# s22s/erased-cells

Measured on AMD Instinct MI355X. Metric: Gcells/s + HBM-GB/s roofline %, u8/u16->f64 16384^2, 1/2/4/8 GPUs, higher is better.
Workload: dtype f64

## Files before the change

### erased-cells_amd/csrc/ec_abi.hip

```cpp
#include <hip/hip_runtime.h>


#include <cfloat>
#include <cstdarg>
#include <cstdio>
#include <cstring>
#include <map>
#include <mutex>
#include <string>

#include "ec_lattice.hpp"
#include "ec_map_kernels.hpp"
#include "ec_reduce_kernels.hpp"
#include "ec_runtime.hpp"

namespace ecd {

static_assert(kMaxReduceBlocks <= kFinalizeMaxParts, "the finalize kernels read at most kFinalizeMaxParts partials");

static ec_status ensure_init() { return ensure_ready(); }

static int64_t* result_words(const Scratch& sc) { return sc.host_dev ? sc.host_dev : sc.dev_result(); }
static ec_status fetch_result(const Scratch& sc, int words, hipStream_t s) {
    if (!sc.host_dev) {
// ... 14 lines not shown
    return st;
}

template <typename K>
static int resident_per_cu(K kernel, int block, int want) {
    int nb = 0;
    if (hipOccupancyMaxActiveBlocksPerMultiprocessor(&nb, kernel, block, 0) != hipSuccess || nb < 1) {
        (void)hipGetLastError();
        return want;
    }
    return nb < want ? nb : want;
}

static unsigned residue(const void* p, size_t mod) { return static_cast<unsigned>(reinterpret_cast<uintptr_t>(p) % mod); }
static ReducePlan plan_reduction(const void* p0, unsigned residue1, size_t cell_size, size_t n, const ReduceShape& shape,
                                 const size_t* stream_bytes, int nstreams) {
    return reduce_plan(residue(p0, 16), residue1, cell_size, n, shape, device_cus(), tuning().reduce_bpc, tuning().unaligned_vector != 0,
                       cache_plan(stream_bytes, nstreams));
}
constexpr ReduceShape kScanShape = {kRBlock, kReduceU, 4, kRBlock, 4};

static inline hipStream_t S(ec_stream s) { return static_cast<hipStream_t>(s); }

template <typename Fn> struct pure_store : std::false_type {};
template <typename W> struct pure_store<FillFn<W>> : std::true_type {};

template <typename Fn, int U>
static void launch_map_u(const Fn& fn, size_t n, hipStream_t s) {
    const size_t groups = n / Fn::CPL;
    const size_t tiles = (groups + size_t(kBlock) * U - 1) / (size_t(kBlock) * U);
    const size_t stream_bytes[2] = {n * Fn::kIn0, n * Fn::kIn1};
    const unsigned lds = (pure_store<Fn>::value ? static_cast<unsigned>(tuning().write_lds_kb.load())
                                                : (Fn::kIn0 != 0 ? static_cast<unsigned>(tuning().map_lds_kb.load()) : 0u)) << 10;
    k_map<Fn, U><<<grid_for(tiles), kBlock, lds, s>>>(fn, n, cache_plan(stream_bytes, 2));
}

template <typename Fn>
static ec_status launch_map(const Fn& fn, size_t n, bool aligned, hipStream_t s, const char* what) {
    if (n == 0) return EC_OK;
    if (!aligned) {
        k_map_cellwise<Fn><<<grid_capped((n + kBlock - 1) / kBlock, 8), kBlock, 0, s>>>(fn, n);
    } else {
        switch (tuning().map_u) {
            case 1: launch_map_u<Fn, 1>(fn, n, s); break;
            case 4: launch_map_u<Fn, 4>(fn, n, s); break;
            default: launch_map_u<Fn, 2>(fn, n, s); break;
        }
    }
    return check_launch(what);
// ... 29 lines not shown
        break;
    switch (st) { EC_WITH_CT(EC_ROW) }
#undef EC_ROW
    return set_error(EC_ERR_UNSUPPORTED_TYPE, "convert: bad dtype");
}

template <typename T>
static ec_status launch_min_max(const void* p, const uint8_t* mask, size_t n, int64_t* keys2_dev, hipStream_t s) {
    Scratch sc;
    ec_status st = get_scratch(s, &sc);
    if (st != EC_OK) return st;
    const T* tp = static_cast<const T*>(p);
    unsigned grid = 0;
    if (n > 0) {
        const size_t stream_bytes[2] = {n * sizeof(T), mask ? n : 0};
        auto launch = [&](auto u_tag, auto block_tag, int per_cu) {
            constexpr int U = decltype(u_tag)::value, BLOCK = decltype(block_tag)::value;
            static const int resident[2] = {resident_per_cu(k_min_max_partials<T, false, U, BLOCK>, BLOCK, per_cu),
                                            resident_per_cu(k_min_max_partials<T, true, U, BLOCK>, BLOCK, per_cu)};
            const ReduceShape shape = {BLOCK, U, resident[mask ? 1 : 0], kBlock, 8};
            const ReducePlan pl = plan_reduction(p, mask ? residue(mask, 16 / sizeof(T)) : 0u, sizeof(T), n, shape, stream_bytes, 2);
            grid = pl.grid;
            int64_t* direct = pl.aligned && pl.single ? keys2_dev : nullptr;
            if (!pl.aligned) {
                if (mask) k_min_max_partials_cellwise<T, true><<<grid, kBlock, 0, s>>>(tp, mask, n, sc.dev);
                else k_min_max_partials_cellwise<T, false><<<grid, kBlock, 0, s>>>(tp, nullptr, n, sc.dev);
            } else if (mask) {
                k_min_max_partials<T, true, U, BLOCK><<<grid, BLOCK, 0, s>>>(tp, mask, n, sc.dev, pl.head_policy, direct);
            } else {
                k_min_max_partials<T, false, U, BLOCK><<<grid, BLOCK, 0, s>>>(tp, nullptr, n, sc.dev, pl.head_policy, direct);
            }
            return direct != nullptr;
        };
        using std::integral_constant;
        bool direct = false;
        switch (tuning().reduce_shape) {
// ... 237 lines not shown
extern "C" ec_status ec_min_max(ec_dtype t, const void* p, const uint8_t* mask_or_null, size_t n, ec_value* mn, ec_value* mx,
                                ec_stream stream) {
    EC_REQUIRE_INIT();
    if (!mn || !mx || (n > 0 && !p)) return set_error(EC_ERR_ARG, "ec_min_max: null pointer");
    int64_t keys2[2];
    ec_status st = sync_result(S(stream), 2, keys2, [&](const Scratch&, int64_t* words) {
        return dispatch_min_max(t, p, mask_or_null, n, words, S(stream));
    });
    if (st != EC_OK) return st;
    return ec_min_max_decode(t, keys2, mn, mx);
}

template <typename W>
static ec_status first_diff_w(const void* l, const void* r, size_t n, const Scratch& sc, hipStream_t s, unsigned* grid_out) {
    const size_t stream_bytes[2] = {n * sizeof(W), n * sizeof(W)};
    const ReducePlan pl = plan_reduction(l, residue(r, 16), sizeof(W), n, kScanShape, stream_bytes, 2);
    k_first_diff_partials<W, kReduceU><<<pl.grid, kRBlock, 0, s>>>(static_cast<const W*>(l), static_cast<const W*>(r), n,
                                                                  reinterpret_cast<uint64_t*>(sc.dev), pl.aligned, pl.head_policy);
    *grid_out = pl.grid;
    return check_launch("first_diff(partials)");
}

extern "C" ec_status ec_first_difference(ec_dtype t, const void* l, const void* r, size_t n, uint64_t* index, ec_stream stream) {
    EC_REQUIRE_INIT();
    if (!ecl::valid(t)) return set_error(EC_ERR_UNSUPPORTED_TYPE, "ec_first_difference: bad dtype %d", int(t));
    if (!index || (n > 0 && (!l || !r))) return set_error(EC_ERR_ARG, "ec_first_difference: null pointer");
    *index = n;
    if (n == 0) return EC_OK;
    int64_t word[2];
    ec_status st = sync_result(S(stream), 1, word, [&](const Scratch& sc, int64_t* words) {
        unsigned grid = 0;
// ... 116 lines not shown
    if (n == 0) return EC_OK;
    if (!m || !out) return set_error(EC_ERR_ARG, "ec_mask_not: null pointer");
    MaskNot fn{m, out};
    return launch_map(fn, n, aligned16(m, out, out), S(stream), "mask_not");
}

extern "C" ec_status ec_mask_counts_device(const uint8_t* m, size_t n, uint64_t* counts2_dev, ec_stream stream) {
    EC_REQUIRE_INIT();
    if (!counts2_dev || (n > 0 && !m)) return set_error(EC_ERR_ARG, "ec_mask_counts_device: null pointer");
    Scratch sc;
    ec_status st = get_scratch(S(stream), &sc);
    if (st != EC_OK) return st;
    unsigned grid = 0;
    if (n > 0) {
        const size_t stream_bytes[1] = {n};
        const ReducePlan pl = plan_reduction(m, 0u, 1, n, kScanShape, stream_bytes, 1);
        grid = pl.grid;
        uint64_t* direct = pl.single ? counts2_dev : nullptr;
        const int one = tuning().counts_one_launch.load();
        uint64_t* acc = (!direct && ((one == 1 && n < (size_t(1) << 29)) || (one >= 2 && n < (size_t(1) << 40)))) ? reinterpret_cast<uint64_t*>(sc.dev_acc()) : nullptr;
        k_mask_count_partials<kReduceU><<<grid, kRBlock, 0, S(stream)>>>(m, n, reinterpret_cast<uint64_t*>(sc.dev), pl.aligned, pl.head_policy,
                                                                        direct, acc, counts2_dev);
        st = check_launch("mask_counts(partials)");
        if (st != EC_OK || direct || acc) return st;
    }
    k_mask_count_finalize<<<1, kFinalizeBlock, 0, S(stream)>>>(reinterpret_cast<const uint64_t*>(sc.dev), static_cast<int>(grid), n, counts2_dev);
    return check_launch("mask_counts(finalize)");
}

extern "C" ec_status ec_mask_counts(const uint8_t* m, size_t n, uint64_t* n_true, uint64_t* n_false, ec_stream stream) {
    EC_REQUIRE_INIT();
// ... 41 lines not shown
```

### erased-cells_amd/csrc/ec_binop_tu.hpp

```cpp
#pragma once

#include <hip/hip_runtime.h>

#include <cmath>

#include "ec_binop_kernels.hpp"
#include "ec_runtime.hpp"

namespace ecd {

static inline unsigned lds_cap(int knob, int rule_kb) { return static_cast<unsigned>(knob >= 0 ? knob : rule_kb) << 10; }

template <typename L, typename R, int OP>
static ec_status launch_binop_pair(const void* l, const void* r, size_t n, double* out, hipStream_t s) {
    const Tuning& tu = tuning();
    const L* lp = static_cast<const L*>(l);
    const R* rp = static_cast<const R*>(r);
    constexpr int U = kBinopU;
    if (!aligned16(l, r, out)) {
        k_binop_cellwise<L, R, OP><<<grid_capped((n + kBlock - 1) / kBlock, 8), kBlock, 0, s>>>(lp, rp, out, n);
        return check_launch("binop(cellwise)");
    }
    constexpr bool kCanStage = Staged<L>::value || Staged<R>::value;
    const int variant = tu.binop_variant.load();
    const size_t stream_bytes[2] = {n * sizeof(L), l == r ? 0 : n * sizeof(R)};
    unsigned policy = cache_plan(stream_bytes, 2, n * sizeof(double));
    if (l == r && (policy & 1u)) policy |= 2u;
    constexpr bool kRulePair = kCanStage && ((sizeof(L) == 8) != (sizeof(R) == 8)) && (sizeof(L) <= 4 || sizeof(R) <= 4);
    const bool by_rule = variant < 0 && kRulePair && policy == 0 && n >= (size_t(1) << 20);
    if (kCanStage && (variant == 1 || by_rule)) {
        const size_t tiles = (n / kLdsWaveCells + kWavesPerBlock - 1) / kWavesPerBlock;
        constexpr unsigned kStatic = kWavesPerBlock * unsigned(Staged<L>::kSlabBytes + Staged<R>::kSlabBytes);
        const int knob = tu.binop_lds_kb.load();
        const unsigned lds = knob >= 0 ? unsigned(knob) << 10 : by_rule ? 32000u - kStatic : 0u;
        k_binop_lds<L, R, OP><<<grid_for(tiles), kBlock, lds, s>>>(lp, rp, out, n);
        if (by_rule) lds_rule_launches().fetch_add(1, std::memory_order_relaxed);
        return check_launch(by_rule ? "binop(lds, by rule)" : "binop(lds)");
    }
    const LoadedStream st[2] = {{l, sizeof(L)}, {r, sizeof(R)}};
    const unsigned head = peel_head(st, 2, n);
    const size_t tiles = (((n - head) >> 1) + size_t(kBlock) * U - 1) / (size_t(kBlock) * U);
    k_binop_direct<L, R, OP, U><<<grid_for(tiles), kBlock, lds_cap(tuning().binop_lds_kb.load(), sizeof(L) == 8 && sizeof(R) == 8 ? 48 : 0), s>>>(lp, rp, out, n, head | (policy << 8));
    return check_launch("binop(direct)");
}
// ... 7 lines not shown
    constexpr int U = kBinopU;
    if (!aligned16(l, r, out) || !aligned16(lm, rm, om)) {
        k_masked_binop_cellwise<L, R, OP><<<grid_capped((n + kBlock - 1) / kBlock, 8), kBlock, 0, s>>>(lp, lm, rp, rm, out, om, n);
        return check_launch("masked_binop(cellwise)");
    }
    constexpr bool kCanStage = Staged<L>::value || Staged<R>::value;
    if (kCanStage && tu.binop_variant == 1) {
        const size_t tiles = (n / kLdsWaveCells + kWavesPerBlock - 1) / kWavesPerBlock;
        k_masked_binop<L, R, OP, U, true><<<grid_for(tiles), kBlock, lds_cap(tu.binop_lds_kb.load(), 0), s>>>(lp, lm, rp, rm, out, om, n, 0u);
        return check_launch("masked_binop(lds)");
    }
    const LoadedStream st[2] = {{l, sizeof(L)}, {r, sizeof(R)}};
    const unsigned head = peel_head(st, 2, n);
    const size_t tiles = (((n - head) >> 1) + size_t(kBlock) * U - 1) / (size_t(kBlock) * U);
    const size_t stream_bytes[4] = {n * sizeof(L), l == r ? 0 : n * sizeof(R), n, lm == rm ? 0 : n};
    unsigned policy = cache_plan(stream_bytes, 4, n * sizeof(double));
    if (l == r && (policy & 1u)) policy |= 2u;
    if (lm == rm && (policy & 4u)) policy |= 8u;
    k_masked_binop<L, R, OP, U, false><<<grid_for(tiles), kBlock, 0, s>>>(lp, lm, rp, rm, out, om, n, head | (policy << 8));
    return check_launch("masked_binop(direct)");
}


template <typename L, int OP>
static ec_status launch_scalar(const void* l, double rhs, size_t n, double* out, hipStream_t s) {
    const L* lp = static_cast<const L*>(l);
    constexpr int U = kBinopU;
    if (!aligned16(l, out, out)) {
        k_binop_scalar_cellwise<L, OP><<<grid_capped((n + kBlock - 1) / kBlock, 8), kBlock, 0, s>>>(lp, rhs, out, n);
        return check_launch("binop_scalar(cellwise)");
    }
    const LoadedStream st[1] = {{l, sizeof(L)}};
    const unsigned head = peel_head(st, 1, n);
    const size_t tiles = (((n - head) >> 1) + size_t(kBlock) * U - 1) / (size_t(kBlock) * U);
    const size_t stream_bytes[1] = {n * sizeof(L)};
    const unsigned policy = cache_plan(stream_bytes, 1, n * sizeof(double));
    const unsigned lds = lds_cap(tuning().scalar_lds_kb.load(), sizeof(L) == 8 ? 32 : 0);
    if constexpr (!is_fp<L>::value) {
        if (std::isfinite(rhs) && !(OP == EC_DIV && rhs == 0.0)) {
            k_binop_scalar_direct<L, OP, U, false><<<grid_for(tiles), kBlock, lds, s>>>(lp, rhs, out, n, head | (policy << 8));
            return check_launch("binop_scalar(direct, no NaN possible)");
        }
    }
    k_binop_scalar_direct<L, OP, U><<<grid_for(tiles), kBlock, lds, s>>>(lp, rhs, out, n, head | (policy << 8));
    return check_launch("binop_scalar(direct)");
}

template <int OP>
ec_status dispatch_binop(int lt, const void* l, int rt, const void* r, size_t n, double* out, hipStream_t s) {
#define EC_ROW(LID, LT)                                                                         \
    case LID:                                                                                   \
// ... 60 lines not shown
```

### erased-cells_amd/csrc/ec_expr.hip

```cpp
#include <hip/hip_runtime.h>

#include <atomic>
#include <cstdlib>
#include <cstring>

#include <limits>
#include <mutex>
#include <string>

#include "ec_expr.hpp"
#include "ec_expr_fixed.hpp"
#include "ec_expr_jit.hpp"
#include "ec_lattice.hpp"
#include "ec_runtime.hpp"

using namespace ecd;

static std::atomic<int64_t> g_interpreted{0};

namespace ecd {
int64_t expr_stat(const char* key, bool* known) {
    if (!std::strcmp(key, "expr_interp_launches")) {
        *known = true;
        return g_interpreted.load(std::memory_order_relaxed);
// ... 42 lines not shown
        for (int j = k + 1; j < n_steps && !read_later; ++j) {
            const int me = kRefReg0 + st.dst;
            if (j > k + 1 && (steps[j].a == me || steps[j].b == me)) read_later = true;
            if (steps[j].dst == st.dst) break;
        }
        if (!read_later) w |= kStepNoFile;
        ea.prog[k >> 2] |= w << (16 * (k & 3));
    }
    ea.nstreams = static_cast<int8_t>(n_streams);
    ea.nsteps = static_cast<int8_t>(n_steps);
    return EC_OK;
}

static ec_status prepare_expr(ExprArgs& ea, bool* aligned_out, int* cls, const ec_dtype* dt, const void* const* p, int32_t n_streams,
                              const uint8_t* const* masks, const ec_value* scalars, int32_t n_scalars, const ec_expr_step* steps,
                              int32_t n_steps, size_t n, const char* what) {
    ec_status pst = program_of(ea, dt, n_streams, n_scalars, steps, n_steps, what);
    if (pst != EC_OK) return pst;
    if (!p || (n_scalars > 0 && !scalars)) return set_error(EC_ERR_ARG, "%s: null pointer", what);
    bool aligned = true;
    LoadedStream st[kExprMaxStreams];
    for (int k = 0; k < n_streams; ++k) {
        if (!p[k]) return set_error(EC_ERR_ARG, "%s: stream %d is null", what, k);
        ea.p[k] = p[k];
        aligned = aligned && aligned_to(p[k], 16);
        st[k] = {p[k], ecl::size_of(dt[k])};
        for (int j = 0; j < k && st[k].same_as < 0; ++j)
            if (p[j] == p[k]) st[k].same_as = j;
        cls[k] = fused_class_index(st[k].size);
    }
    for (int k = n_streams; k < kExprMaxStreams; ++k) ea.p[k] = p[0];
    for (int k = 0; k < n_scalars; ++k) {
        if (!ecl::valid(scalars[k].dtype)) return set_error(EC_ERR_ARG, "%s: bad dtype of scalar %d", what, k);
        ea.sc[k] = ec_value_to_f64(&scalars[k]);
    }
    if (masks)
        for (int k = 0; k < n_streams; ++k) {
            const ec_status mst = add_mask(masks[k], k, what, ea.m, &ea.nmask, &aligned);
            if (mst != EC_OK) return mst;
        }
    *aligned_out = aligned;
    ea.head = static_cast<uint8_t>(peel_head(st, n_streams, n));
    ea.cacheable = static_cast<uint8_t>(stream_policy(st, ea.nmask, n));
    return EC_OK;
}

static ec_status launch_expr(const ec_dtype* dt, const void* const* p, int32_t n_streams, const uint8_t* const* masks,
                             const ec_value* scalars, int32_t n_scalars, const ec_expr_step* steps, int32_t n_steps, size_t n,
                             double* out, uint8_t* out_mask, hipStream_t s, const char* what) {
    ExprArgs ea{};
    bool aligned = true;
    int cls[kExprMaxStreams] = {0, 0, 0, 0};
    if (!out) return set_error(EC_ERR_ARG, "%s: null pointer", what);
    if (masks && !out_mask) return set_error(EC_ERR_ARG, "%s: null out_mask", what);
    ec_status pst = prepare_expr(ea, &aligned, cls, dt, p, n_streams, masks, scalars, n_scalars, steps, n_steps, n, what);
    if (pst != EC_OK) return pst;
    aligned = aligned && aligned_to(out, 16) && (!masks || aligned_to(out_mask, 16));
    if (!aligned) {
        ea.head = 0;
        k_expr_cellwise<0><<<grid_capped((n + kBlock - 1) / kBlock, 8), kBlock, 0, s>>>(ea, out, out_mask, n);
        return check_launch("expr(cellwise)");
    }
    bool fixed = false;
    ec_status fst = expr_fixed_launch(ea, n, out, out_mask, s, &fixed);
    if (fst != EC_OK) return fst;
    if (fixed) return check_launch("expr(ahead-of-time)");
    bool compiled = false;
    ec_status jst = expr_jit_launch(ea, n, out, out_mask, nullptr, s, &compiled);
    if (jst != EC_OK) return jst;
    if (compiled) return check_launch("expr(compiled)");
// ... 32 lines not shown

static ec_status expr_min_max_keys(const ec_dtype* dt, const void* const* p, const uint8_t* const* masks_or_null, int32_t n_streams,
                                   const ec_value* scalars, int32_t n_scalars, const ec_expr_step* steps, int32_t n_steps, size_t n,
                                   int64_t* keys2_dev, hipStream_t s, const char* what) {
    ec_status st;
    {
        ExprArgs probe{};
        if ((st = program_of(probe, dt, n_streams, n_scalars, steps, n_steps, what)) != EC_OK) return st;
    }
    if (!keys2_dev) return set_error(EC_ERR_ARG, "%s: null keys", what);
    if ((st = check_hip(hipMemcpyAsync(keys2_dev, kF64Identities, sizeof kF64Identities, hipMemcpyHostToDevice, s), "hipMemcpyAsync(keys)")) != EC_OK) return st;
    if (n == 0) return EC_OK;
    ExprArgs ea{};
    bool aligned = true;
    int cls[kExprMaxStreams] = {0, 0, 0, 0};
    if ((st = prepare_expr(ea, &aligned, cls, dt, p, n_streams, masks_or_null, scalars, n_scalars, steps, n_steps, n, what)) != EC_OK) return st;
    if (aligned) {
        bool compiled = false;
        if ((st = expr_jit_launch(ea, n, nullptr, nullptr, keys2_dev, s, &compiled)) != EC_OK) return st;
        if (compiled) return EC_OK;
    }
    void *tmp = nullptr, *tmask = nullptr;
    if ((st = ec_alloc_async(&tmp, n * sizeof(double), s)) != EC_OK) return st;
    if (masks_or_null && (st = ec_alloc_async(&tmask, n, s)) != EC_OK) {
        (void)ec_free_async(tmp, s);
        return st;
    }
    st = launch_expr(dt, p, n_streams, masks_or_null, scalars, n_scalars, steps, n_steps, n, static_cast<double*>(tmp), static_cast<uint8_t*>(tmask), s, what);
    if (st == EC_OK) st = ec_min_max_keys(EC_F64, tmp, static_cast<const uint8_t*>(tmask), n, keys2_dev, s);
    const std::string keep = st != EC_OK ? last_error_text() : std::string();
    (void)ec_free_async(tmp, s);
// ... 64 lines not shown
```

### erased-cells_amd/csrc/ec_fused.hip

```cpp
#include <hip/hip_runtime.h>

#include "ec_fused_any.hpp"
#include "ec_lattice.hpp"

using namespace ecd;

static ec_status launch_fused_any(FusedArgs& fa, int nops, size_t n, double* out, uint8_t* out_mask, hipStream_t s) {
    LoadedStream st[4];
    int cls[4];
    bool small = fa.o2 == EC_DIV && (fa.o1 == EC_ADD || fa.o1 == EC_SUB) && (fa.o3 == EC_ADD || fa.o3 == EC_SUB || fa.o3 == kOpNone);
    for (int k = 0; k < 4; ++k) {
        if (k < nops && !fa.is_sc[k] && fa.alias[k] == k) st[k] = {fa.p[k], ecl::size_of(fa.dt[k])};
        cls[k] = fused_class_index(st[k].size);
        if (k < nops) small = small && !fa.is_sc[k] && ecl::is_integral(fa.dt[k]) && ecl::size_of(fa.dt[k]) <= 2;
    }
    fa.small = small ? 1 : 0;
    fa.head = static_cast<uint8_t>(peel_head(st, 4, n));
    fa.cacheable = static_cast<uint8_t>(stream_policy(st, fa.nmask, n));
    FusedAnyKernel kern = nullptr;
    switch (cls[0]) {
        case 0: kern = fused_any_kernel<0>(cls[1], cls[2], cls[3]); break;
        case 1: kern = fused_any_kernel<1>(cls[1], cls[2], cls[3]); break;
        case 2: kern = fused_any_kernel<2>(cls[1], cls[2], cls[3]); break;
        case 3: kern = fused_any_kernel<4>(cls[1], cls[2], cls[3]); break;
        default: kern = fused_any_kernel<8>(cls[1], cls[2], cls[3]); break;
    }
    if (!kern) return set_error(EC_ERR_ARG, "ec_fused: no kernel for load classes %d %d %d %d", cls[0], cls[1], cls[2], cls[3]);
    launch_stream_tile<kFusedU>(kern, fa.head, n, s, fa, out, out_mask, n);
    return check_launch("fused(any)");
}

static ec_status launch_fused(int o1, int o2, int o3, const ec_dtype dt[4], const void* const p[4],
                              const uint8_t* const masks[4], const ec_value* scalars, size_t n, double* out,
// ... 89 lines not shown
```

### erased-cells_amd/csrc/ec_runtime.hip

```cpp
#include <hip/hip_runtime.h>

#include <atomic>
#include <cstdarg>
#include <cstdint>
#include <cstdio>
#include <cstdlib>
#include <cstring>
#include <map>
#include <memory>
#include <mutex>
#include <string>

#include "ec_hostpipe.hpp"
#include "ec_runtime.hpp"

namespace ecd {

static thread_local std::string t_err;
static thread_local int t_narrow_src = -1, t_narrow_dst = -1;

ec_status set_error(ec_status code, const char* fmt, ...) {
    char buf[512];
    va_list ap;
    va_start(ap, fmt);
// ... 55 lines not shown
    int device = -1;
    int cus = 256;
    hipMemPool_t pool = nullptr;
    std::map<hipStream_t, ScratchEntry> scratch;
};

constexpr size_t kMaxScratchPerDevice = 64;

static std::mutex g_mu;
static std::map<int, DeviceState> g_devs;
static std::atomic<int> g_default_device{-1};
static std::atomic<uint64_t> g_generation{1};
static std::atomic<uint64_t> g_stamp{0};
static std::atomic<int64_t> g_lds_rule_launches{0};
std::atomic<int64_t>& lds_rule_launches() { return g_lds_rule_launches; }
static std::atomic<int64_t> g_pool_allocs{0};
static Tuning g_tuning;

static thread_local int t_device = -1;
static thread_local uint64_t t_generation = 0;
static thread_local int t_active = -1;
static thread_local int t_cus = 256;

int64_t expr_stat(const char* key, bool* known);
void expr_jit_release();
Tuning& tuning() { return g_tuning; }

namespace {
enum class Out { Clamp, Refuse, Bool };
struct Knob {
    const char* key;
    std::atomic<int>* i;
    std::atomic<int64_t>* l;
    int64_t lo, hi;
    Out out;
    bool pow2 = false;
};
constexpr int64_t kMaxMiB = int64_t(1) << 20;
const Knob kKnobs[] = {
    {"binop_variant", &g_tuning.binop_variant, nullptr, -1, 1, Out::Refuse},
    {"reduce_bpc", &g_tuning.reduce_bpc, nullptr, 0, kMaxReduceBlocks, Out::Clamp},
// ... 335 lines not shown
    }
    return EC_OK;
}

extern "C" ec_status ec_stream_destroy(ec_stream s) {
    ec_status st = ec_release_stream(s);
    if (st != EC_OK) return st;
    return check_hip(hipStreamDestroy(S(s)), "hipStreamDestroy");
}
extern "C" ec_status ec_stream_sync(ec_stream s) { return check_hip(hipStreamSynchronize(S(s)), "hipStreamSynchronize"); }

extern "C" ec_status ec_stat_get(const char* key, int64_t* value) {
    if (!key || !value) return set_error(EC_ERR_ARG, "ec_stat_get: null argument");
    if (!std::strcmp(key, "pool_allocs")) *value = g_pool_allocs.load(std::memory_order_relaxed);
    else if (!std::strcmp(key, "binop_lds_rule_launches")) *value = g_lds_rule_launches.load(std::memory_order_relaxed);
    else if (!std::strncmp(key, "tune.", 5)) {
        const Knob* kn = knob_of(key + 5);
        if (!kn) return set_error(EC_ERR_ARG, "ec_stat_get: unknown knob '%s'", key + 5);
        *value = kn->i ? int64_t(kn->i->load()) : kn->l->load();
    } else if (!std::strcmp(key, "devices")) {
        std::lock_guard<std::mutex> lk(g_mu);
        *value = static_cast<int64_t>(g_devs.size());
    } else if (!std::strcmp(key, "scratch_streams")) {
        std::lock_guard<std::mutex> lk(g_mu);
        int64_t n = 0;
        for (auto& kv : g_devs) n += static_cast<int64_t>(kv.second.scratch.size());
        *value = n;
    } else {
        bool known = false;
        *value = expr_stat(key, &known);
// ... 26 lines not shown
```

### erased-cells_amd/csrc/ec_runtime.hpp

```cpp
#pragma once

#include <hip/hip_runtime.h>
#include <stddef.h>
#include <stdint.h>

#include <atomic>
#include <memory>
#include <mutex>
#include <string>

#include "ec_reduce_plan.hpp"
#include "erased_cells.h"

namespace ecd {

constexpr int kBinopU = 2;

struct Tuning;
Tuning& tuning();
struct Tuning {
    std::atomic<int> binop_variant{-1};
    std::atomic<int> reduce_bpc{0};
    std::atomic<int> reduce_shape{0};
    std::atomic<int> map_u{2};
    std::atomic<int> peel{1};
// ... 11 lines not shown
    std::atomic<int> fused_lds_kb{0};
    std::atomic<int> counts_one_launch{1};
    std::atomic<int> cache_force{-1};
    std::atomic<int64_t> pool_keep_mb{32768};
};

int device_cus();
int current_device();

ec_status ensure_ready();
ec_status set_error(ec_status code, const char* fmt, ...);
ec_status set_error_text(ec_status code, const std::string& text);
const std::string& last_error_text();
ec_status set_narrowing(int src, int dst);
std::atomic<int64_t>& lds_rule_launches();
ec_status check_launch(const char* what);
ec_status check_hip(hipError_t e, const char* what);

class DeviceScope {
    int32_t before_ = -1;
    const bool had_;

public:
    DeviceScope() : had_(ec_get_device(&before_) == EC_OK) {}
    DeviceScope(const DeviceScope&) = delete;
    DeviceScope& operator=(const DeviceScope&) = delete;
    ~DeviceScope() {
        if (!had_ || current_device() == before_) return;
        const std::string keep = last_error_text();
        (void)ec_set_device(before_);
// ... 16 lines not shown
struct LoadedStream {
    const void* p = nullptr;
    size_t size = 0;
    int same_as = -1;
};
inline unsigned peel_head(const LoadedStream* st, int count, size_t n) {
    if (n < 2 || !tuning().peel) return 0;
    unsigned c0 = 0, c1 = 0;
    for (int k = 0; k < count; ++k) {
        c0 += peel_cost(st[k].p, st[k].size, 0);
        c1 += peel_cost(st[k].p, st[k].size, 1);
    }
    return c1 < c0 ? 1u : 0u;
}

inline unsigned cache_plan(const size_t* bytes, int n, size_t value_out_bytes = 0) {
    const int forced = tuning().cache_force.load();
    if (forced >= 0) return static_cast<unsigned>(forced) & ((1u << (n < 8 ? n : 8)) - 1u);
    const size_t budget = static_cast<size_t>(tuning().mall_mb.load()) << 20;
    unsigned plan = 0;
    size_t used = 0, largest_taken = 0;
    bool taken[8] = {false, false, false, false, false, false, false, false};
    for (int round = 0; round < n && n <= 8; ++round) {
        int best = -1;
        for (int k = 0; k < n; ++k)
            if (!taken[k] && bytes[k] > 0 && (best < 0 || bytes[k] < bytes[best])) best = k;
        if (best < 0 || used + bytes[best] > budget) break;
        taken[best] = true;
        used += bytes[best];
        if (bytes[best] > largest_taken) largest_taken = bytes[best];
        plan |= 1u << best;
    }
    if (value_out_bytes > 0 && plan != 0)
        for (int k = 0; k < n && n <= 8; ++k)
            if (!taken[k] && bytes[k] > 0 && bytes[k] <= largest_taken) return 0;
    return plan;
}

inline unsigned stream_policy(const LoadedStream (&st)[4], int nmask, size_t n) {
    size_t bytes[8] = {0, 0, 0, 0, 0, 0, 0, 0};
    for (int k = 0; k < 4; ++k) bytes[k] = st[k].same_as < 0 ? n * st[k].size : 0;
    for (int j = 0; j < nmask; ++j) bytes[4 + j] = n;
    unsigned policy = cache_plan(bytes, 8, n * sizeof(double));
    for (int k = 0; k < 4; ++k)
        if (st[k].same_as >= 0) policy = (policy & ~(1u << k)) | (((policy >> st[k].same_as) & 1u) << k);
    return policy;
}

inline ec_status add_mask(const uint8_t* m, int k, const char* what, const uint8_t** ms, int8_t* nmask, bool* aligned) {
    if (!m) return set_error(EC_ERR_ARG, "%s: null mask %d", what, k);
    for (int j = 0; j < *nmask; ++j)
        if (ms[j] == m) return EC_OK;
    ms[(*nmask)++] = m;
    *aligned = *aligned && aligned_to(m, 16);
    return EC_OK;
}

inline unsigned grid_for(size_t tiles) {
// ... 31 lines not shown
```

### erased-cells_amd/csrc/ec_window.hip

```cpp
#include <hip/hip_runtime.h>

#include "ec_lattice.hpp"
#include "ec_runtime.hpp"
#include "ec_window_checks.hpp"
#include "ec_window_kernels.hpp"

namespace ecd {

static bool make_axis(uint64_t win, uint64_t out, WindowAxis* a) {
    a->q = win / out;
    a->r = win % out;
    a->out = out;
    if (out > (UINT64_MAX >> 2)) return false;
    const unsigned __int128 worst = (unsigned __int128)(2 * out) * a->r + win;
    if (worst > UINT64_MAX) return false;
    const uint64_t num = a->q * out + a->r;
    a->d0 = num / (2 * out);
    a->rem0 = num % (2 * out);
    return true;
}

static bool rows_aligned(const void* raster, const WindowGeom& g, size_t cell, const void* contiguous) {
    return ((reinterpret_cast<uintptr_t>(raster) + g.origin * cell) | (g.pitch * cell) | (g.w * cell) | reinterpret_cast<uintptr_t>(contiguous)) % 16 == 0;
}

template <int W, bool MASKED>
static ec_status launch_window(int kind, const WindowArgs& args, const WindowAxis* ax, const WindowAxis* ay, bool vector, hipStream_t s) {
    WindowArgs a = args;
    const size_t bytes[2] = {a.g.n * W, MASKED ? a.g.n : 0};
    a.cacheable = cache_plan(bytes, 2);
    if (!vector) {
        const uint64_t chunks = ((a.g.w + kBlock - 1) / kBlock) * (a.g.n / a.g.w);
        const WindowAxis id_x{1, 0, a.g.w, 0, a.g.w}, id_y{1, 0, a.g.n / a.g.w, 0, a.g.n / a.g.w};
        if (kind == kWinPut) k_window_cellwise<W, MASKED, true><<<grid_capped(chunks, 8), kBlock, 0, s>>>(a, id_x, id_y);
        else k_window_cellwise<W, MASKED, false><<<grid_capped(chunks, 8), kBlock, 0, s>>>(a, ax ? *ax : id_x, ay ? *ay : id_y);
        return check_launch("window(cell-wise)");
    }
    const uint64_t slots = (a.g.n + (16 / W) - 1) / (16 / W), per_tile = uint64_t(kBlock) * kWindowU;
    const unsigned grid = grid_for((slots + per_tile - 1) / per_tile);
    if (uint64_t(grid) * per_tile < slots) return set_error(EC_ERR_ARG, "window: more than 2^31 tiles");
    if (ax) k_window_nearest<W, MASKED><<<grid, kBlock, 0, s>>>(a, *ax, *ay);
    else if (kind == kWinPut) k_window_put<W, MASKED><<<grid, kBlock, 0, s>>>(a);
    else k_window_copy<W, MASKED><<<grid, kBlock, 0, s>>>(a);
    return check_launch(ax ? "window(nearest)" : kind == kWinPut ? "window(put)" : "window(copy)");
}
// ... 53 lines not shown
```

### erased-cells_amd/csrc/ec_window_resample.hip

```cpp
#include <hip/hip_runtime.h>

#include "ec_window_checks.hpp"
#include "ec_window_resample_kernels.hpp"

namespace ecd {

typedef unsigned __int128 u128;

static uint64_t gcd_u64(uint64_t a, uint64_t b) {
    while (b) {
        const uint64_t t = a % b;
        a = b;
        b = t;
    }
    return a;
}

static const char* make_resample_axis(int32_t alg, uint64_t win, uint64_t out, ResampleAxis* a) {
    if (alg == EC_RESAMPLE_AVERAGE) {
        if ((u128)win * out > UINT64_MAX) return "win * out";
        const uint64_t g = gcd_u64(win, out);
        *a = ResampleAxis{win / g, 0, out / g, win / g, 0, win - 1, 0, 0, 0, 0};
    } else {
        if ((u128)2 * out * win + out > UINT64_MAX) return "2 * out * win + out";
// ... 4 lines not shown
    a->c0 = a->add / a->den;
    a->f0 = a->add % a->den;
    return nullptr;
}

static uint64_t resample_tiles(uint64_t n, size_t cell) {
    const uint64_t per_slot = 16 / cell, slots = n / per_slot + (n % per_slot != 0), per_tile = uint64_t(kBlock) * kWindowU;
    return slots / per_tile + (slots % per_tile != 0);
}

template <typename T, bool MASKED>
static ec_status launch_resample(const ResampleArgs& args, uint64_t win_cells, hipStream_t s) {
    constexpr size_t W = sizeof(T);
    ResampleArgs a = args;
    const size_t bytes[2] = {win_cells * W, MASKED ? win_cells : 0};
    a.w.cacheable = cache_plan(bytes, 2);
    k_window_resample<T, MASKED><<<grid_for(resample_tiles(a.w.g.n, W)), kBlock, 0, s>>>(a);
    return check_launch("window(resample)");
}

static ec_status dispatch_resample(ec_dtype t, const ResampleArgs& a, uint64_t win_cells, hipStream_t s) {
    const bool masked = a.w.in_mask != nullptr;
    switch (t) {
#define X(code, T) \
    case code: return masked ? launch_resample<T, true>(a, win_cells, s) : launch_resample<T, false>(a, win_cells, s);
        EC_WITH_CT(X)
#undef X
        default: return set_error(EC_ERR_UNSUPPORTED_TYPE, "ec_window_resample: bad dtype %d", int(t));
    }
}

// ... 39 lines not shown
```

Before: 611.7.

## Admit reads to MALL cache only when the same buffer was recently read

Adds a per-device host-side ledger that tracks recently read address ranges, with a byte counter standing in for cache pressure. A stream is marked cacheable in the last-level cache only if the same range was read recently enough to still fit in the budget. Streams seen for the first time are read with the non-caching policy. This aims to keep one-shot streaming reads from polluting the MALL while keeping reuse across calls. The cost is a mutex and ring scan on the host for every launch, and cache decisions now depend on call history, with the ledger bypassed during graph capture.

Result: no change. 614.8, median of 6 (+0.5%).

```diff
diff --git a/erased-cells_amd/csrc/ec_abi.hip b/erased-cells_amd/csrc/ec_abi.hip
--- a/erased-cells_amd/csrc/ec_abi.hip
+++ b/erased-cells_amd/csrc/ec_abi.hip
@@ -52,9 +52,9 @@
 
 static unsigned residue(const void* p, size_t mod) { return static_cast<unsigned>(reinterpret_cast<uintptr_t>(p) % mod); }
 static ReducePlan plan_reduction(const void* p0, unsigned residue1, size_t cell_size, size_t n, const ReduceShape& shape,
-                                 const size_t* stream_bytes, int nstreams) {
+                                 const size_t* stream_bytes, const void* const* stream_base, int nstreams, hipStream_t s) {
     return reduce_plan(residue(p0, 16), residue1, cell_size, n, shape, device_cus(), tuning().reduce_bpc, tuning().unaligned_vector != 0,
-                       cache_plan(stream_bytes, nstreams));
+                       cache_plan(stream_bytes, stream_base, nstreams, s));
 }
 constexpr ReduceShape kScanShape = {kRBlock, kReduceU, 4, kRBlock, 4};
 
@@ -62,6 +62,14 @@
 
 template <typename Fn> struct pure_store : std::false_type {};
 template <typename W> struct pure_store<FillFn<W>> : std::true_type {};
+
+template <typename Fn> static void map_inputs(const Fn&, const void* (&)[2]) { static_assert(Fn::kIn0 == 0 && Fn::kIn1 == 0, "name the Fn's inputs"); }
+template <typename Sx, typename Dx> static void map_inputs(const ConvertFn<Sx, Dx>& f, const void* (&p)[2]) { p[0] = f.src; }
+template <typename T> static void map_inputs(const NegFn<T>& f, const void* (&p)[2]) { p[0] = f.src; }
+template <typename W> static void map_inputs(const MaskFromNodataFn<W>& f, const void* (&p)[2]) { p[0] = f.src; }
+template <typename W> static void map_inputs(const MaskSelectFn<W>& f, const void* (&p)[2]) { p[0] = f.src, p[1] = f.mask; }
+template <int KIND> static void map_inputs(const MaskBin<KIND>& f, const void* (&p)[2]) { p[0] = f.l, p[1] = f.r; }
+static void map_inputs(const MaskNot& f, const void* (&p)[2]) { p[0] = f.m; }
 
 template <typename Fn, int U>
 static void launch_map_u(const Fn& fn, size_t n, hipStream_t s) {
@@ -70,7 +78,9 @@
     const size_t stream_bytes[2] = {n * Fn::kIn0, n * Fn::kIn1};
     const unsigned lds = (pure_store<Fn>::value ? static_cast<unsigned>(tuning().write_lds_kb.load())
                                                 : (Fn::kIn0 != 0 ? static_cast<unsigned>(tuning().map_lds_kb.load()) : 0u)) << 10;
-    k_map<Fn, U><<<grid_for(tiles), kBlock, lds, s>>>(fn, n, cache_plan(stream_bytes, 2));
+    const void* stream_base[2] = {nullptr, nullptr};
+    map_inputs(fn, stream_base);
+    k_map<Fn, U><<<grid_for(tiles), kBlock, lds, s>>>(fn, n, cache_plan(stream_bytes, stream_base, 2, s));
 }
 
 template <typename Fn>
@@ -130,12 +140,13 @@
     unsigned grid = 0;
     if (n > 0) {
         const size_t stream_bytes[2] = {n * sizeof(T), mask ? n : 0};
+        const void* const stream_base[2] = {p, mask};
         auto launch = [&](auto u_tag, auto block_tag, int per_cu) {
             constexpr int U = decltype(u_tag)::value, BLOCK = decltype(block_tag)::value;
             static const int resident[2] = {resident_per_cu(k_min_max_partials<T, false, U, BLOCK>, BLOCK, per_cu),
                                             resident_per_cu(k_min_max_partials<T, true, U, BLOCK>, BLOCK, per_cu)};
             const ReduceShape shape = {BLOCK, U, resident[mask ? 1 : 0], kBlock, 8};
-            const ReducePlan pl = plan_reduction(p, mask ? residue(mask, 16 / sizeof(T)) : 0u, sizeof(T), n, shape, stream_bytes, 2);
+            const ReducePlan pl = plan_reduction(p, mask ? residue(mask, 16 / sizeof(T)) : 0u, sizeof(T), n, shape, stream_bytes, stream_base, 2, s);
             grid = pl.grid;
             int64_t* direct = pl.aligned && pl.single ? keys2_dev : nullptr;
             if (!pl.aligned) {
@@ -403,7 +414,8 @@
 template <typename W>
 static ec_status first_diff_w(const void* l, const void* r, size_t n, const Scratch& sc, hipStream_t s, unsigned* grid_out) {
     const size_t stream_bytes[2] = {n * sizeof(W), n * sizeof(W)};
-    const ReducePlan pl = plan_reduction(l, residue(r, 16), sizeof(W), n, kScanShape, stream_bytes, 2);
+    const void* const stream_base[2] = {l, r};
+    const ReducePlan pl = plan_reduction(l, residue(r, 16), sizeof(W), n, kScanShape, stream_bytes, stream_base, 2, s);
     k_first_diff_partials<W, kReduceU><<<pl.grid, kRBlock, 0, s>>>(static_cast<const W*>(l), static_cast<const W*>(r), n,
                                                                   reinterpret_cast<uint64_t*>(sc.dev), pl.aligned, pl.head_policy);
     *grid_out = pl.grid;
@@ -550,7 +562,8 @@
     unsigned grid = 0;
     if (n > 0) {
         const size_t stream_bytes[1] = {n};
-        const ReducePlan pl = plan_reduction(m, 0u, 1, n, kScanShape, stream_bytes, 1);
+        const void* const stream_base[1] = {m};
+        const ReducePlan pl = plan_reduction(m, 0u, 1, n, kScanShape, stream_bytes, stream_base, 1, S(stream));
         grid = pl.grid;
         uint64_t* direct = pl.single ? counts2_dev : nullptr;
         const int one = tuning().counts_one_launch.load();
diff --git a/erased-cells_amd/csrc/ec_binop_tu.hpp b/erased-cells_amd/csrc/ec_binop_tu.hpp
--- a/erased-cells_amd/csrc/ec_binop_tu.hpp
+++ b/erased-cells_amd/csrc/ec_binop_tu.hpp
@@ -24,10 +24,12 @@
     constexpr bool kCanStage = Staged<L>::value || Staged<R>::value;
     const int variant = tu.binop_variant.load();
     const size_t stream_bytes[2] = {n * sizeof(L), l == r ? 0 : n * sizeof(R)};
-    unsigned policy = cache_plan(stream_bytes, 2, n * sizeof(double));
+    const void* const stream_base[2] = {l, r};
+    unsigned by_size = 0;
+    unsigned policy = cache_plan(stream_bytes, stream_base, 2, s, n * sizeof(double), &by_size);
     if (l == r && (policy & 1u)) policy |= 2u;
     constexpr bool kRulePair = kCanStage && ((sizeof(L) == 8) != (sizeof(R) == 8)) && (sizeof(L) <= 4 || sizeof(R) <= 4);
-    const bool by_rule = variant < 0 && kRulePair && policy == 0 && n >= (size_t(1) << 20);
+    const bool by_rule = variant < 0 && kRulePair && by_size == 0 && n >= (size_t(1) << 20);
     if (kCanStage && (variant == 1 || by_rule)) {
         const size_t tiles = (n / kLdsWaveCells + kWavesPerBlock - 1) / kWavesPerBlock;
         constexpr unsigned kStatic = kWavesPerBlock * unsigned(Staged<L>::kSlabBytes + Staged<R>::kSlabBytes);
@@ -65,7 +67,8 @@
     const unsigned head = peel_head(st, 2, n);
     const size_t tiles = (((n - head) >> 1) + size_t(kBlock) * U - 1) / (size_t(kBlock) * U);
     const size_t stream_bytes[4] = {n * sizeof(L), l == r ? 0 : n * sizeof(R), n, lm == rm ? 0 : n};
-    unsigned policy = cache_plan(stream_bytes, 4, n * sizeof(double));
+    const void* const stream_base[4] = {l, r, lm, rm};
+    unsigned policy = cache_plan(stream_bytes, stream_base, 4, s, n * sizeof(double));
     if (l == r && (policy & 1u)) policy |= 2u;
     if (lm == rm && (policy & 4u)) policy |= 8u;
     k_masked_binop<L, R, OP, U, false><<<grid_for(tiles), kBlock, 0, s>>>(lp, lm, rp, rm, out, om, n, head | (policy << 8));
@@ -85,7 +88,8 @@
     const unsigned head = peel_head(st, 1, n);
     const size_t tiles = (((n - head) >> 1) + size_t(kBlock) * U - 1) / (size_t(kBlock) * U);
     const size_t stream_bytes[1] = {n * sizeof(L)};
-    const unsigned policy = cache_plan(stream_bytes, 1, n * sizeof(double));
+    const void* const stream_base[1] = {l};
+    const unsigned policy = cache_plan(stream_bytes, stream_base, 1, s, n * sizeof(double));
     const unsigned lds = lds_cap(tuning().scalar_lds_kb.load(), sizeof(L) == 8 ? 32 : 0);
     if constexpr (!is_fp<L>::value) {
         if (std::isfinite(rhs) && !(OP == EC_DIV && rhs == 0.0)) {
diff --git a/erased-cells_amd/csrc/ec_cache_ledger.hpp b/erased-cells_amd/csrc/ec_cache_ledger.hpp
--- /dev/null
+++ b/erased-cells_amd/csrc/ec_cache_ledger.hpp
@@ -0,0 +1,96 @@
+#pragma once
+
+#include <stddef.h>
+#include <stdint.h>
+
+#include <mutex>
+
+namespace ecd {
+
+inline unsigned plan_by_size(const size_t* bytes, int n, size_t value_out_bytes, size_t budget) {
+    unsigned plan = 0;
+    size_t used = 0, largest_taken = 0;
+    bool taken[8] = {false, false, false, false, false, false, false, false};
+    for (int round = 0; round < n && n <= 8; ++round) {
+        int best = -1;
+        for (int k = 0; k < n; ++k)
+            if (!taken[k] && bytes[k] > 0 && (best < 0 || bytes[k] < bytes[best])) best = k;
+        if (best < 0 || used + bytes[best] > budget) break;
+        taken[best] = true;
+        used += bytes[best];
+        if (bytes[best] > largest_taken) largest_taken = bytes[best];
+        plan |= 1u << best;
+    }
+    if (value_out_bytes > 0 && plan != 0)
+        for (int k = 0; k < n && n <= 8; ++k)
+            if (!taken[k] && bytes[k] > 0 && bytes[k] <= largest_taken) return 0;
+    return plan;
+}
+
+struct ReadRange {
+    uintptr_t base = 0;
+    size_t span = 0;
+};
+
+constexpr int kLedgerRing = 32;
+
+class CacheLedger {
+public:
+    unsigned admit(unsigned plan, const size_t* bytes, const ReadRange* range, int n, size_t budget, unsigned* declined = nullptr) {
+        std::lock_guard<std::mutex> lk(mu_);
+        unsigned seen = 0;
+        uint64_t candidates = 0;
+        for (int k = 0; k < n && k < 8; ++k) {
+            if (!(plan >> k & 1u)) continue;
+            candidates += bytes[k];
+            if (seen_locked(range[k], budget)) seen |= 1u << k;
+        }
+        for (int k = 0; k < n && k < 8; ++k)
+            if (range[k].span > 0) stamp_locked(range[k]);
+        counter_ += candidates;
+        if (declined) *declined = plan & ~seen;
+        return seen;
+    }
+    uint64_t counter() const {
+        std::lock_guard<std::mutex> lk(mu_);
+        return counter_;
+    }
+
+private:
+    struct Entry {
+        uintptr_t base = 0;
+        size_t span = 0;
+        uint64_t stamp = 0;
+    };
+    bool seen_locked(const ReadRange& r, size_t budget) const {
+        if (r.span == 0) return false;
+        for (const Entry& e : ring_)
+            if (e.span >= r.span && e.base <= r.base && r.base - e.base <= e.span - r.span && counter_ - e.stamp <= budget) return true;
+        return false;
+    }
+    void stamp_locked(const ReadRange& r) {
+        for (Entry& e : ring_)
+            if (e.span == r.span && e.base == r.base) {
+                e.stamp = counter_;
+                return;
+            }
+        ring_[next_] = Entry{r.base, r.span, counter_};
+        next_ = (next_ + 1) % kLedgerRing;
+    }
+
+    mutable std::mutex mu_;
+    Entry ring_[kLedgerRing];
+    int next_ = 0;
+    uint64_t counter_ = 0;
+};
+
+inline unsigned plan_launch(CacheLedger* ledger, const size_t* bytes, const ReadRange* range, int n, size_t value_out_bytes, size_t budget,
+                            unsigned* by_size = nullptr, unsigned* declined = nullptr) {
+    const unsigned plan = plan_by_size(bytes, n, value_out_bytes, budget);
+    if (by_size) *by_size = plan;
+    if (declined) *declined = 0;
+    if (!ledger || n > 8) return plan;
+    return ledger->admit(plan, bytes, range, n, budget, declined);
+}
+
+}
diff --git a/erased-cells_amd/csrc/ec_expr.hip b/erased-cells_amd/csrc/ec_expr.hip
--- a/erased-cells_amd/csrc/ec_expr.hip
+++ b/erased-cells_amd/csrc/ec_expr.hip
@@ -80,7 +80,7 @@
 
 static ec_status prepare_expr(ExprArgs& ea, bool* aligned_out, int* cls, const ec_dtype* dt, const void* const* p, int32_t n_streams,
                               const uint8_t* const* masks, const ec_value* scalars, int32_t n_scalars, const ec_expr_step* steps,
-                              int32_t n_steps, size_t n, const char* what) {
+                              int32_t n_steps, size_t n, hipStream_t s, const char* what) {
     ec_status pst = program_of(ea, dt, n_streams, n_scalars, steps, n_steps, what);
     if (pst != EC_OK) return pst;
     if (!p || (n_scalars > 0 && !scalars)) return set_error(EC_ERR_ARG, "%s: null pointer", what);
@@ -107,7 +107,7 @@
         }
     *aligned_out = aligned;
     ea.head = static_cast<uint8_t>(peel_head(st, n_streams, n));
-    ea.cacheable = static_cast<uint8_t>(stream_policy(st, ea.nmask, n));
+    ea.cacheable = static_cast<uint8_t>(stream_policy(st, ea.m, ea.nmask, n, s));
     return EC_OK;
 }
 
@@ -119,7 +119,7 @@
     int cls[kExprMaxStreams] = {0, 0, 0, 0};
     if (!out) return set_error(EC_ERR_ARG, "%s: null pointer", what);
     if (masks && !out_mask) return set_error(EC_ERR_ARG, "%s: null out_mask", what);
-    ec_status pst = prepare_expr(ea, &aligned, cls, dt, p, n_streams, masks, scalars, n_scalars, steps, n_steps, n, what);
+    ec_status pst = prepare_expr(ea, &aligned, cls, dt, p, n_streams, masks, scalars, n_scalars, steps, n_steps, n, s, what);
     if (pst != EC_OK) return pst;
     aligned = aligned && aligned_to(out, 16) && (!masks || aligned_to(out_mask, 16));
     if (!aligned) {
@@ -182,7 +182,7 @@
     ExprArgs ea{};
     bool aligned = true;
     int cls[kExprMaxStreams] = {0, 0, 0, 0};
-    if ((st = prepare_expr(ea, &aligned, cls, dt, p, n_streams, masks_or_null, scalars, n_scalars, steps, n_steps, n, what)) != EC_OK) return st;
+    if ((st = prepare_expr(ea, &aligned, cls, dt, p, n_streams, masks_or_null, scalars, n_scalars, steps, n_steps, n, s, what)) != EC_OK) return st;
     if (aligned) {
         bool compiled = false;
         if ((st = expr_jit_launch(ea, n, nullptr, nullptr, keys2_dev, s, &compiled)) != EC_OK) return st;
diff --git a/erased-cells_amd/csrc/ec_fused.hip b/erased-cells_amd/csrc/ec_fused.hip
--- a/erased-cells_amd/csrc/ec_fused.hip
+++ b/erased-cells_amd/csrc/ec_fused.hip
@@ -16,7 +16,7 @@
     }
     fa.small = small ? 1 : 0;
     fa.head = static_cast<uint8_t>(peel_head(st, 4, n));
-    fa.cacheable = static_cast<uint8_t>(stream_policy(st, fa.nmask, n));
+    fa.cacheable = static_cast<uint8_t>(stream_policy(st, fa.m, fa.nmask, n, s));
     FusedAnyKernel kern = nullptr;
     switch (cls[0]) {
         case 0: kern = fused_any_kernel<0>(cls[1], cls[2], cls[3]); break;
diff --git a/erased-cells_amd/csrc/ec_runtime.hip b/erased-cells_amd/csrc/ec_runtime.hip
--- a/erased-cells_amd/csrc/ec_runtime.hip
+++ b/erased-cells_amd/csrc/ec_runtime.hip
@@ -93,6 +93,10 @@
 static std::atomic<uint64_t> g_stamp{0};
 static std::atomic<int64_t> g_lds_rule_launches{0};
 std::atomic<int64_t>& lds_rule_launches() { return g_lds_rule_launches; }
+static CacheLedger g_cache_ledgers[32];
+static std::atomic<int64_t> g_cache_admitted{0}, g_cache_declined_unseen{0};
+std::atomic<int64_t>& cache_admitted_streams() { return g_cache_admitted; }
+std::atomic<int64_t>& cache_declined_unseen_streams() { return g_cache_declined_unseen; }
 static std::atomic<int64_t> g_pool_allocs{0};
 static Tuning g_tuning;
 
@@ -104,6 +108,16 @@
 int64_t expr_stat(const char* key, bool* known);
 void expr_jit_release();
 Tuning& tuning() { return g_tuning; }
+CacheLedger& cache_ledger() { return g_cache_ledgers[static_cast<unsigned>(t_active < 0 ? 0 : t_active) % 32u]; }
+bool stream_is_capturing(hipStream_t s) {
+    if (!s) return false;
+    hipStreamCaptureStatus cap = hipStreamCaptureStatusNone;
+    if (hipStreamIsCapturing(s, &cap) != hipSuccess) {
+        (void)hipGetLastError();
+        return true;
+    }
+    return cap != hipStreamCaptureStatusNone;
+}
 
 namespace {
 enum class Out { Clamp, Refuse, Bool };
@@ -469,6 +483,8 @@
     if (!key || !value) return set_error(EC_ERR_ARG, "ec_stat_get: null argument");
     if (!std::strcmp(key, "pool_allocs")) *value = g_pool_allocs.load(std::memory_order_relaxed);
     else if (!std::strcmp(key, "binop_lds_rule_launches")) *value = g_lds_rule_launches.load(std::memory_order_relaxed);
+    else if (!std::strcmp(key, "cache_admitted_streams")) *value = g_cache_admitted.load(std::memory_order_relaxed);
+    else if (!std::strcmp(key, "cache_declined_unseen_streams")) *value = g_cache_declined_unseen.load(std::memory_order_relaxed);
     else if (!std::strncmp(key, "tune.", 5)) {
         const Knob* kn = knob_of(key + 5);
         if (!kn) return set_error(EC_ERR_ARG, "ec_stat_get: unknown knob '%s'", key + 5);
diff --git a/erased-cells_amd/csrc/ec_runtime.hpp b/erased-cells_amd/csrc/ec_runtime.hpp
--- a/erased-cells_amd/csrc/ec_runtime.hpp
+++ b/erased-cells_amd/csrc/ec_runtime.hpp
@@ -9,6 +9,7 @@
 #include <mutex>
 #include <string>
 
+#include "ec_cache_ledger.hpp"
 #include "ec_reduce_plan.hpp"
 #include "erased_cells.h"
 
@@ -50,6 +51,10 @@
 const std::string& last_error_text();
 ec_status set_narrowing(int src, int dst);
 std::atomic<int64_t>& lds_rule_launches();
+CacheLedger& cache_ledger();
+std::atomic<int64_t>& cache_admitted_streams();
+std::atomic<int64_t>& cache_declined_unseen_streams();
+bool stream_is_capturing(hipStream_t s);
 ec_status check_launch(const char* what);
 ec_status check_hip(hipError_t e, const char* what);
 
@@ -96,34 +101,40 @@
     return c1 < c0 ? 1u : 0u;
 }
 
-inline unsigned cache_plan(const size_t* bytes, int n, size_t value_out_bytes = 0) {
+inline ReadRange read_range(const void* p, size_t span) { return ReadRange{reinterpret_cast<uintptr_t>(p), span}; }
+inline unsigned cache_plan(const size_t* bytes, const ReadRange* range, int n, hipStream_t s, size_t value_out_bytes = 0, unsigned* by_size = nullptr) {
     const int forced = tuning().cache_force.load();
-    if (forced >= 0) return static_cast<unsigned>(forced) & ((1u << (n < 8 ? n : 8)) - 1u);
+    unsigned plan = 0;
+    if (forced >= 0) {
+        plan = static_cast<unsigned>(forced) & ((1u << (n < 8 ? n : 8)) - 1u);
+        if (by_size) *by_size = plan;
+        return plan;
+    }
     const size_t budget = static_cast<size_t>(tuning().mall_mb.load()) << 20;
-    unsigned plan = 0;
-    size_t used = 0, largest_taken = 0;
-    bool taken[8] = {false, false, false, false, false, false, false, false};
-    for (int round = 0; round < n && n <= 8; ++round) {
-        int best = -1;
-        for (int k = 0; k < n; ++k)
-            if (!taken[k] && bytes[k] > 0 && (best < 0 || bytes[k] < bytes[best])) best = k;
-        if (best < 0 || used + bytes[best] > budget) break;
-        taken[best] = true;
-        used += bytes[best];
-        if (bytes[best] > largest_taken) largest_taken = bytes[best];
-        plan |= 1u << best;
-    }
-    if (value_out_bytes > 0 && plan != 0)
-        for (int k = 0; k < n && n <= 8; ++k)
-            if (!taken[k] && bytes[k] > 0 && bytes[k] <= largest_taken) return 0;
-    return plan;
+    unsigned declined = 0;
+    const unsigned seen = plan_launch(stream_is_capturing(s) ? nullptr : &cache_ledger(), bytes, range, n, value_out_bytes, budget, by_size, &declined);
+    if (seen) cache_admitted_streams().fetch_add(__builtin_popcount(seen), std::memory_order_relaxed);
+    if (declined) cache_declined_unseen_streams().fetch_add(__builtin_popcount(declined), std::memory_order_relaxed);
+    return seen;
+}
+inline unsigned cache_plan(const size_t* bytes, const void* const* p, int n, hipStream_t s, size_t value_out_bytes = 0, unsigned* by_size = nullptr) {
+    ReadRange range[8];
+    for (int k = 0; k < n && k < 8; ++k) range[k] = read_range(p[k], bytes[k]);
+    return cache_plan(bytes, range, n, s, value_out_bytes, by_size);
 }
 
-inline unsigned stream_policy(const LoadedStream (&st)[4], int nmask, size_t n) {
+inline unsigned stream_policy(const LoadedStream (&st)[4], const uint8_t* const* m, int nmask, size_t n, hipStream_t s) {
     size_t bytes[8] = {0, 0, 0, 0, 0, 0, 0, 0};
-    for (int k = 0; k < 4; ++k) bytes[k] = st[k].same_as < 0 ? n * st[k].size : 0;
-    for (int j = 0; j < nmask; ++j) bytes[4 + j] = n;
-    unsigned policy = cache_plan(bytes, 8, n * sizeof(double));
+    const void* p[8] = {nullptr, nullptr, nullptr, nullptr, nullptr, nullptr, nullptr, nullptr};
+    for (int k = 0; k < 4; ++k) {
+        bytes[k] = st[k].same_as < 0 ? n * st[k].size : 0;
+        p[k] = st[k].p;
+    }
+    for (int j = 0; j < nmask; ++j) {
+        bytes[4 + j] = n;
+        p[4 + j] = m[j];
+    }
+    unsigned policy = cache_plan(bytes, p, 8, s, n * sizeof(double));
     for (int k = 0; k < 4; ++k)
         if (st[k].same_as >= 0) policy = (policy & ~(1u << k)) | (((policy >> st[k].same_as) & 1u) << k);
     return policy;
diff --git a/erased-cells_amd/csrc/ec_window.hip b/erased-cells_amd/csrc/ec_window.hip
--- a/erased-cells_amd/csrc/ec_window.hip
+++ b/erased-cells_amd/csrc/ec_window.hip
@@ -28,7 +28,11 @@
 static ec_status launch_window(int kind, const WindowArgs& args, const WindowAxis* ax, const WindowAxis* ay, bool vector, hipStream_t s) {
     WindowArgs a = args;
     const size_t bytes[2] = {a.g.n * W, MASKED ? a.g.n : 0};
-    a.cacheable = cache_plan(bytes, 2);
+    const uint64_t win_w = ax ? ax->q * ax->out + ax->r : a.g.w, win_h = ay ? ay->q * ay->out + ay->r : a.g.n / a.g.w;
+    const uint64_t first = kind == kWinPut ? 0 : a.g.origin, cells = kind == kWinPut ? a.g.n : (win_h - 1) * a.g.pitch + win_w;
+    const ReadRange range[2] = {read_range(static_cast<const char*>(a.in) + first * W, cells * W),
+                                read_range(MASKED ? a.in_mask + first : nullptr, MASKED ? cells : 0)};
+    a.cacheable = cache_plan(bytes, range, 2, s);
     if (!vector) {
         const uint64_t chunks = ((a.g.w + kBlock - 1) / kBlock) * (a.g.n / a.g.w);
         const WindowAxis id_x{1, 0, a.g.w, 0, a.g.w}, id_y{1, 0, a.g.n / a.g.w, 0, a.g.n / a.g.w};
diff --git a/erased-cells_amd/csrc/ec_window_resample.hip b/erased-cells_amd/csrc/ec_window_resample.hip
--- a/erased-cells_amd/csrc/ec_window_resample.hip
+++ b/erased-cells_amd/csrc/ec_window_resample.hip
@@ -42,7 +42,10 @@
     constexpr size_t W = sizeof(T);
     ResampleArgs a = args;
     const size_t bytes[2] = {win_cells * W, MASKED ? win_cells : 0};
-    a.w.cacheable = cache_plan(bytes, 2);
+    const uint64_t cells = a.ay.last * a.w.g.pitch + a.ax.last + 1;
+    const ReadRange range[2] = {read_range(static_cast<const char*>(a.w.in) + a.w.g.origin * W, cells * W),
+                                read_range(MASKED ? a.w.in_mask + a.w.g.origin : nullptr, MASKED ? cells : 0)};
+    a.w.cacheable = cache_plan(bytes, range, 2, s);
     k_window_resample<T, MASKED><<<grid_for(resample_tiles(a.w.g.n, W)), kBlock, 0, s>>>(a);
     return check_launch("window(resample)");
 }
```
